# gildas-lormeau/zlib-streams-ts

Measured on NVIDIA B200. Metric: deflate_input_GBps, higher is better.
Workload: dtype u8

## Files before the change

### zlib-streams-ts_b200/csrc/zs_lz77.cu

```cuda
#include <cstdio>
#include <cstdlib>

#include "zs_common.cuh"

namespace {

#ifndef ZS_SEARCH_WARPS
#define ZS_SEARCH_WARPS 30
#endif
#ifndef ZS_HASH_BITS
#define ZS_HASH_BITS 14
#endif
#ifndef ZS_LZ_PREV_POS
#define ZS_LZ_PREV_DELTA 1
#endif
constexpr int kSearchWarps = ZS_SEARCH_WARPS;
constexpr int kWarpParse = kSearchWarps;
constexpr int kWarpInsert = kSearchWarps + 1;
constexpr int kThreads = 32 * (kSearchWarps + 2);
constexpr int kStep = 32 * kSearchWarps;
constexpr unsigned kMaxDist = 32768u - 2u * kStep;
constexpr unsigned kNoPrev = 0xffffu;
constexpr unsigned kSymLimit = 16383u;
constexpr unsigned kTooFar = 4096u;
constexpr unsigned kHashBits = ZS_HASH_BITS;
constexpr unsigned kRing = 65536;
constexpr unsigned kRingGuard = 288;
constexpr unsigned pow2_at_least(unsigned v) { unsigned r = 1; while (r < v) r <<= 1; return r; }
constexpr unsigned kResRing = pow2_at_least(4 * kStep + 64);
constexpr unsigned kMjRing = pow2_at_least(3 * kStep + 64);
constexpr unsigned kPbRing = pow2_at_least(2 * kSearchWarps + 4);
constexpr unsigned kMaxSegChunks = 256;

struct LevelCfg { int lazy_fn, good, lazy, nice, chain; };
__constant__ LevelCfg c_levels[10] = {
    {0, 0, 0, 0, 0},      {0, 4, 4, 8, 4},      {0, 4, 5, 16, 8},      {0, 4, 6, 32, 32},
    {1, 4, 4, 16, 16},    {1, 8, 16, 32, 32},   {1, 8, 16, 128, 128},  {1, 8, 32, 128, 256},
    {1, 32, 128, 258, 1024}, {1, 32, 258, 258, 4096}};

constexpr uint32_t PREP_HAS_PRED = 1u << 21, PREP_LAST = 1u << 22, PREP_VALID = 1u << 23;

struct Smem {
    uint8_t ring[kRing + kRingGuard];
    uint16_t head[1 << kHashBits];
    uint16_t prev[32768];
    uint32_t prep[3 * kStep];
    uint16_t oldh[2 * kStep];
    uint2 pb[kPbRing];
    uint32_t res[kResRing];
    uint2 mj[kMjRing];
    uint32_t bnd[kMaxSegChunks + 1];
    uint32_t seg;
    uint32_t claim[2];
    alignas(8) uint64_t stage_bar;
};
static_assert(sizeof(Smem) <= 227 * 1024, "shared memory budget");

struct LzArgs {
    const uint8_t* buf;
    uint64_t org;
    uint64_t valid_lo;
    uint64_t data_end;
    const uint64_t* in_off;
    uint32_t n_chunks, seg_chunks, n_seg, max_bpc;
    uint32_t n_big, seg_small;
    int level;
    int strategy;
    int cross;
    uint32_t* sym;
    uint32_t* chunk_nblk;
    uint32_t* blk_desc;
    uint32_t* seg_counter;
    int debug;
    unsigned stop_after, stop_active;
};

#ifdef ZS_LZ_PROF
__device__ unsigned long long g_prof[16];
#define PROF_T(i) if (lane == 0) atomicAdd(&g_prof[i], (unsigned long long)(clock64() - t_begin))
#else
#define PROF_T(i)
#endif

__device__ __forceinline__ unsigned res_slot(uint32_t q) { return q & (kResRing - 1u); }
__device__ __forceinline__ unsigned mj_slot(uint32_t q) { return q & (kMjRing - 1u); }

__device__ __forceinline__ uint32_t win32(const Smem& S, uint64_t pos) {
    const unsigned idx = (unsigned)pos & (kRing - 1u);
    const unsigned al = idx & ~3u;
    const uint32_t lo = *reinterpret_cast<const uint32_t*>(S.ring + al);
    const uint32_t hi = *reinterpret_cast<const uint32_t*>(S.ring + al + 4);
    return __funnelshift_r(lo, hi, (idx & 3u) * 8u);
}

__device__ __forceinline__ void stage_window(Smem& S, const LzArgs& a, uint64_t from, uint64_t to, unsigned tid, unsigned nthr) {
    const uint64_t safe16 = (a.data_end + 15) & ~15ull;
    for (uint64_t pos = from + 16ull * tid; pos < to; pos += 16ull * nthr) {
        uint4 v = make_uint4(0, 0, 0, 0);
        if (pos < safe16) v = __ldg(reinterpret_cast<const uint4*>(a.buf + pos));
        const unsigned idx = (unsigned)pos & (kRing - 1u);
        *reinterpret_cast<uint4*>(S.ring + idx) = v;
        if (idx < kRingGuard) *reinterpret_cast<uint4*>(S.ring + kRing + idx) = v;
    }
}

#ifndef ZS_LZ_NO_BULK
#define ZS_LZ_BULK 1
#endif
__device__ __forceinline__ unsigned smem_addr(const void* p) { return (unsigned)__cvta_generic_to_shared(p); }
__device__ __forceinline__ void mbar_init(uint64_t* bar, unsigned count) {
    asm volatile("mbarrier.init.shared::cta.b64 [%0], %1;" ::"r"(smem_addr(bar)), "r"(count) : "memory");
    asm volatile("fence.mbarrier_init.release.cluster;" ::: "memory");
}
__device__ __forceinline__ void mbar_expect_tx(uint64_t* bar, unsigned bytes) {
    asm volatile("mbarrier.arrive.expect_tx.shared::cta.b64 _, [%0], %1;" ::"r"(smem_addr(bar)), "r"(bytes) : "memory");
}
__device__ __forceinline__ void mbar_wait(uint64_t* bar, unsigned parity) {
    asm volatile(
        "{\n"
        ".reg .pred p;\n"
        "ZS_MBAR_WAIT:\n"
        "mbarrier.try_wait.parity.shared::cta.b64 p, [%0], %1;\n"
        "@p bra ZS_MBAR_DONE;\n"
        "bra ZS_MBAR_WAIT;\n"
        "ZS_MBAR_DONE:\n"
        "}\n" ::"r"(smem_addr(bar)), "r"(parity) : "memory");
}
__device__ __forceinline__ void bulk_g2s(void* dst, const void* src, unsigned bytes, uint64_t* bar) {
    asm volatile("cp.async.bulk.shared::cluster.global.mbarrier::complete_tx::bytes [%0], [%1], %2, [%3];" ::"r"(smem_addr(dst)),
                 "l"(src), "r"(bytes), "r"(smem_addr(bar))
                 : "memory");
}
__device__ __forceinline__ unsigned bulk_stage(Smem& S, const uint8_t* buf, uint64_t from, uint64_t to) {
    unsigned total = 0;
    while (from < to) {
        const unsigned idx = (unsigned)from & (kRing - 1u);
        unsigned nb = (unsigned)(to - from);
        if (idx + nb > kRing) nb = kRing - idx;
#ifdef ZS_DEBUG_HOOKS
        if (idx + nb > kRing || (nb & 15u) || (idx & 15u) || ((uintptr_t)(buf + from) & 15u)) { printf("[lz77 bulk] bad copy idx %u nb %u\n", idx, nb); __trap(); }
#endif
        bulk_g2s(S.ring + idx, buf + from, nb, &S.stage_bar);
        total += nb;
        if (idx < kRingGuard) {
            const unsigned g = idx + nb < kRingGuard ? nb : kRingGuard - idx;
#ifdef ZS_DEBUG_HOOKS
            if (idx + g > kRingGuard || (g & 15u)) { printf("[lz77 bulk] bad guard copy idx %u g %u\n", idx, g); __trap(); }
#endif
            bulk_g2s(S.ring + kRing + idx, buf + from, g, &S.stage_bar);
            total += g;
        }
        from += nb;
    }
    return total;
}

__device__ __forceinline__ unsigned hash3(uint32_t w) { return ((w & 0xffffffu) * 0x9E3779B1u) >> (32 - kHashBits); }

struct RangeCtx {
    uint32_t cb;
    uint32_t n;
    uint32_t pre;
    uint32_t tail;
    uint32_t q_data;
    uint32_t nc;
    int cross;
    unsigned min_len;
};

__device__ __forceinline__ uint32_t prep_batch(const Smem& S, const RangeCtx& c, uint32_t q0, uint32_t limit) {
    const unsigned lane = zs_lane();
    const uint32_t q = q0 + lane;
    const bool valid = q < limit && q + 2 < c.tail;
    unsigned h = 0;
    if (valid) h = hash3(win32(S, c.cb + q));
#ifndef ZS_PREP_MATCH_ANY
    unsigned peers = __ballot_sync(ZS_FULL_MASK, valid);
#pragma unroll
    for (int bit = 0; bit < (int)kHashBits; ++bit) {
        const bool one = (h >> bit) & 1u;
        const unsigned bal = __ballot_sync(ZS_FULL_MASK, one);
        peers &= one ? bal : ~bal;
    }
#else
    const unsigned peers = __match_any_sync(ZS_FULL_MASK, valid ? h : 0x10000u + lane);
#endif
    if (!valid) return 0u;
    const unsigned lower = peers & zs_lanemask_lt();
    uint32_t w = h | PREP_VALID;
    if (lower) w |= PREP_HAS_PRED | ((31u - __clz(lower)) << 16);
    if ((peers >> lane) == 1u) w |= PREP_LAST;
    return w;
}

__device__ __forceinline__ void head_exchange(Smem& S, uint32_t p16, uint32_t w, uint16_t* oldh) {
    const unsigned h = w & 0x7fffu;
    unsigned old = 0;
    if ((w & PREP_VALID) && !(w & PREP_HAS_PRED)) old = S.head[h];
    if (w & PREP_LAST) S.head[h] = (uint16_t)(p16 + zs_lane());
    oldh[zs_lane()] = (uint16_t)old;
    __syncwarp();
}
__device__ __forceinline__ void link_batch(Smem& S, const RangeCtx& c, uint32_t q0, uint32_t w, unsigned old) {
    if (w & PREP_VALID) {
        const uint32_t q = q0 + zs_lane();
        const unsigned p16 = (c.cb + q) & 0xffffu;
#ifdef ZS_LZ_PREV_DELTA
        unsigned hop = kNoPrev;
        if (w & PREP_HAS_PRED) {
            hop = zs_lane() - ((w >> 16) & 31u);
        } else {
            const unsigned delta = (p16 - old) & 0xffffu;
            if (delta != 0 && delta <= kMaxDist && delta <= q + c.pre) hop = delta;
        }
        S.prev[p16 & 32767u] = (uint16_t)hop;
#else
        unsigned pred = p16;
        if (w & PREP_HAS_PRED) {
            pred = (c.cb + q0 + ((w >> 16) & 31u)) & 0xffffu;
        } else {
            const unsigned delta = (p16 - old) & 0xffffu;
            if (delta != 0 && delta <= kMaxDist && delta <= q + c.pre) pred = (p16 - delta) & 0xffffu;
        }
        S.prev[p16 & 32767u] = (uint16_t)pred;
#endif
    }
}

#ifdef ZS_LZ_PREV_DELTA
__device__ __forceinline__ bool chain_hop(const Smem& S, unsigned& ci, unsigned& dist, unsigned max_back, unsigned& delta) {
    delta = S.prev[ci & 32767u];
    dist += delta;
    if (dist > max_back) return false;
    ci = (ci - delta) & (kRing - 1u);
    return true;
}
#else
__device__ __forceinline__ bool chain_hop(const Smem& S, unsigned& ci, unsigned& dist, unsigned max_back, unsigned& delta) {
    delta = (ci - S.prev[ci & 32767u]) & 0xffffu;
    if (delta == 0) return false;
    dist += delta;
    if (dist > max_back) return false;
    ci = (ci - delta) & (kRing - 1u);
    return true;
}
#endif

__device__ __forceinline__ uint32_t ring32(const Smem& S, unsigned idx) {
    idx &= kRing - 1u;
    const unsigned al = idx & ~3u;
    const uint32_t lo = *reinterpret_cast<const uint32_t*>(S.ring + al);
    const uint32_t hi = *reinterpret_cast<const uint32_t*>(S.ring + al + 4);
    return __funnelshift_r(lo, hi, (idx & 3u) * 8u);
}
__device__ __forceinline__ unsigned first_diff_byte(uint32_t x) { return (unsigned)(__ffs((int)x) - 1) >> 3; }

__device__ __forceinline__ uint2 ring64(const Smem& S, unsigned idx) {
    idx &= kRing - 1u;
    const unsigned al = idx & ~3u, sh = (idx & 3u) * 8u;
    const uint32_t w0 = *reinterpret_cast<const uint32_t*>(S.ring + al);
    const uint32_t w1 = *reinterpret_cast<const uint32_t*>(S.ring + al + 4);
    const uint32_t w2 = *reinterpret_cast<const uint32_t*>(S.ring + al + 8);
    return make_uint2(__funnelshift_r(w0, w1, sh), __funnelshift_r(w1, w2, sh));
}
__device__ __forceinline__ unsigned extend_match(const Smem& S, unsigned ci, unsigned pi, unsigned len, unsigned max_len) {
    unsigned aa = ((ci + len) & (kRing - 1u)) & ~3u, ab = ((pi + len) & (kRing - 1u)) & ~3u;
    const unsigned sa = ((ci + len) & 3u) * 8u, sb = ((pi + len) & 3u) * 8u;
    uint32_t a0 = *reinterpret_cast<const uint32_t*>(S.ring + aa);
    uint32_t b0 = *reinterpret_cast<const uint32_t*>(S.ring + ab);
// ... 140 lines not shown
    if (best_len < c.min_len) return lit;
    if (best_len == 3 && best_dist > kTooFar) return lit;
    return lit | (best_len << 15) | best_dist;
}

constexpr unsigned MJ_MATCH = 1u << 9;
__device__ __forceinline__ unsigned mj_exit(unsigned y) { return y & 0x1ffu; }
__device__ __forceinline__ unsigned mj_count(unsigned y) { return (y >> 10) & 0x3fu; }
__device__ __forceinline__ unsigned mj_pair_exit(unsigned y) { return ((y >> 16) & 0x1ffu) + 32u; }
__device__ __forceinline__ unsigned mj_pair_count(unsigned y) { return y >> 25; }

template <int kMode>
__device__ __forceinline__ void resolve_one(const Smem& S, const LevelCfg& cfg, uint32_t n, uint32_t q0, unsigned& M,
                                            unsigned& J, bool& is_match) {
    const unsigned lane = zs_lane();
    const uint32_t q = q0 + lane;
    const uint32_t r = q < n ? S.res[res_slot(q)] : 0u;
    const unsigned L = (r >> 15) & 0x1ffu;
    unsigned Ln = __shfl_down_sync(ZS_FULL_MASK, L, 1);
    if (lane == 31) Ln = (q + 1 < n) ? ((S.res[res_slot(q + 1)] >> 15) & 0x1ffu) : 0u;
    const bool deferred = kMode == 1 && L >= 3 && L < (unsigned)cfg.lazy && Ln > L;
    is_match = L >= 3 && !deferred;
    J = q < n ? lane + (is_match ? L : 1u) : 32u;
    M = q < n ? 1u << lane : 0u;
#pragma unroll
    for (int round = 0; round < 5; ++round) {
        const unsigned src = J < 32 ? J : lane;
        const unsigned Mj = __shfl_sync(ZS_FULL_MASK, M, src);
        const unsigned Jj = __shfl_sync(ZS_FULL_MASK, J, src);
        if (J < 32) { M |= Mj; J = Jj; }
    }
}

template <int kMode>
__device__ __forceinline__ void resolve_pair(Smem& S, const LevelCfg& cfg, uint32_t n, uint32_t q0) {
    const unsigned lane = zs_lane();
    unsigned Ma, Ja, Mb, Jb;
    bool ma, mb;
    resolve_one<kMode>(S, cfg, n, q0, Ma, Ja, ma);
    resolve_one<kMode>(S, cfg, n, q0 + 32, Mb, Jb, mb);
    const unsigned ca = __popc(Ma), cb = __popc(Mb);
    const unsigned xa = Ja - 32u;
    const unsigned src = xa < 32u ? xa : lane;
    const unsigned jb = __shfl_sync(ZS_FULL_MASK, Jb, src), cbx = __shfl_sync(ZS_FULL_MASK, cb, src);
    const unsigned pair_exit = xa < 32u ? 32u + jb : Ja;
    const unsigned pair_cnt = xa < 32u ? ca + cbx : ca;
    const unsigned pe = pair_exit >= 32u ? pair_exit - 32u : 0u;
    if (q0 + lane < n)
        S.mj[mj_slot(q0 + lane)] = make_uint2(Ma, Ja | (ma ? MJ_MATCH : 0u) | (ca << 10) | (pe << 16) | (pair_cnt << 25));
    if (q0 + 32 + lane < n)
        S.mj[mj_slot(q0 + 32 + lane)] = make_uint2(Mb, Jb | (mb ? MJ_MATCH : 0u) | (cb << 10));
}

struct ParseState {
    uint32_t ppos;
    uint32_t skip;
    uint32_t nsym;
    uint32_t blk;
    uint32_t blk_sym0;
    uint32_t blk_pos0;
    uint32_t jc;
    uint32_t cstart;
    uint32_t nb;
};

__device__ __forceinline__ void close_block(const LzArgs& a, const RangeCtx& rc, ParseState& ps, uint32_t c0, uint32_t pos_end) {
    if (ps.blk < a.max_bpc && zs_lane() == 0) {
        uint32_t* d = a.blk_desc + ((uint64_t)(c0 + ps.jc) * a.max_bpc + ps.blk) * 4;
        d[0] = ps.blk_sym0 - (ps.cstart - rc.q_data);
        d[1] = ps.nsym - ps.blk_sym0;
        d[2] = ps.blk_pos0 - ps.cstart;
        d[3] = pos_end - ps.blk_pos0;
    }
    ps.blk++;
    ps.blk_sym0 = ps.nsym;
    ps.blk_pos0 = pos_end;
}

__device__ __forceinline__ void close_chunk(const Smem& S, const LzArgs& a, const RangeCtx& rc, ParseState& ps, uint32_t c0) {
    close_block(a, rc, ps, c0, ps.nb);
    if (zs_lane() == 0) a.chunk_nblk[c0 + ps.jc] = ps.blk < a.max_bpc ? ps.blk : a.max_bpc;
    ps.jc++;
    ps.cstart = ps.nb;
    ps.nb = ps.jc < rc.nc ? S.bnd[ps.jc + 1] : 0xffffffffu;
    ps.blk = 0;
}

__device__ __forceinline__ unsigned below(unsigned b) { return b >= 32u ? 0xffffffffu : (1u << b) - 1u; }

constexpr int kParseGroup = 16;
template <bool kBoundary>
__device__ __forceinline__ void parse_group(Smem& S, const LzArgs& a, const RangeCtx& rc, ParseState& ps, uint32_t c0,
                                            uint32_t qb, int np) {
    const unsigned lane = zs_lane();
    const uint32_t n = rc.n;
    unsigned ya[kParseGroup], yb[kParseGroup];
#pragma unroll
    for (int u = 0; u < kParseGroup; ++u) {
        const uint32_t q = qb + 64u * u + lane;
        ya[u] = (u < np && q < n) ? S.mj[mj_slot(q)].y : (32u | (32u << 16));
        yb[u] = (u < np && q + 32 < n) ? S.mj[mj_slot(q + 32)].y : 32u;
    }
#pragma unroll
    for (int u = 0; u < kParseGroup; ++u) {
        if (u < np) {
            const uint32_t q0 = qb + 64u * u;
            unsigned entry = 64u;
            const uint32_t first_sym = ps.nsym;
            if (ps.skip >= 64) {
                ps.skip -= 64;
            } else {
                unsigned s = ps.skip;
                entry = s;
                while (kBoundary && ps.nb < q0 + 64u) {
                    const unsigned b = ps.nb - q0;
                    unsigned c;
                    if (b <= s) {
                        c = 0;
                    } else if (s < 32u) {
                        const uint2 m = S.mj[mj_slot(q0 + s)];
                        c = __popc(m.x & below(b));
                        if (b > 32u) {
                            const unsigned xa = mj_exit(m.y) - 32u;
                            if (xa < b - 32u) c += __popc(S.mj[mj_slot(q0 + 32u + xa)].x & below(b - 32u));
                        }
                    } else {
                        c = __popc(S.mj[mj_slot(q0 + s)].x & below(b - 32u));
                    }
                    if (ps.nsym - ps.blk_sym0 + c > kSymLimit) close_block(a, rc, ps, c0, q0 + s);
                    ps.nsym += c;
                    close_chunk(S, a, rc, ps, c0);
                    s = b;
                }
                const unsigned wa = __shfl_sync(ZS_FULL_MASK, ya[u], s & 31u);
                const unsigned wb = __shfl_sync(ZS_FULL_MASK, yb[u], s & 31u);
                unsigned cnt, exit_rel;
                if (s < 32) { cnt = mj_pair_count(wa); exit_rel = mj_pair_exit(wa); }
                else { cnt = mj_count(wb); exit_rel = 32u + mj_exit(wb); }
                if (ps.nsym - ps.blk_sym0 + cnt > kSymLimit) close_block(a, rc, ps, c0, q0 + s);
                ps.nsym += cnt;
                ps.skip = exit_rel >= 64u ? exit_rel - 64u : 0u;
                while (kBoundary && ps.nb <= q0 + exit_rel) close_chunk(S, a, rc, ps, c0);
            }
            if (lane == 0) S.pb[(q0 >> 6) & (kPbRing - 1u)] = make_uint2(entry, first_sym);
        }
    }
}

__device__ __forceinline__ void emit_batch(const Smem& S, const LzArgs& a, uint64_t sym_base, uint32_t n, uint32_t q0) {
    const unsigned lane = zs_lane();
    const uint2 e = S.pb[(q0 >> 6) & (kPbRing - 1u)];
    if (e.x >= 64u) return;
    unsigned entry, first = e.y;
    if (!(q0 & 32u)) {
        if (e.x >= 32u) return;
        entry = e.x;
    } else if (e.x >= 32u) {
        entry = e.x - 32u;
    } else {
        const unsigned ya = S.mj[mj_slot(q0 - 32u + e.x)].y;
        const unsigned xa = mj_exit(ya) - 32u;
        if (xa >= 32u) return;
        entry = xa;
        first += mj_count(ya);
    }
    if (q0 + entry >= n) return;
    const unsigned visited = S.mj[mj_slot(q0 + entry)].x;
    if (((visited >> lane) & 1u) && q0 + lane < n) {
        const uint32_t q = q0 + lane;
        const uint32_t r = S.res[res_slot(q)];
        const bool is_match = (S.mj[mj_slot(q)].y & MJ_MATCH) != 0;
        a.sym[sym_base + first + __popc(visited & zs_lanemask_lt())] =
            is_match ? (((r & 0x7fffu) << 16) | ((r >> 15) & 0x1ffu)) : (r >> 24);
    }
}

__device__ __forceinline__ uint32_t resolved_frontier(uint32_t searched, uint32_t n) {
    if (searched >= n) return n;
    return searched >= 64 ? (searched - 1) & ~63u : 0;
}

template <int kMode>
__global__ void __launch_bounds__(kThreads, 1) lz77_kernel(LzArgs a) {
    extern __shared__ __align__(16) unsigned char smem_raw[];
    Smem& S = *reinterpret_cast<Smem*>(smem_raw);
    const unsigned wid = threadIdx.x >> 5, lane = zs_lane();
    LevelCfg cfg = c_levels[a.level];
    const StopCfg stop = {a.stop_after, a.stop_active};
    (void)stop;
#ifdef ZS_LZ_PROF
    if (a.debug >> 8) cfg.chain = a.debug >> 8;
#endif

#ifdef ZS_LZ_BULK
    if (threadIdx.x == 0) mbar_init(&S.stage_bar, 1);
#endif
    for (;;) {
        if (threadIdx.x == 0) S.seg = atomicAdd(a.seg_counter, 1u);
        __syncthreads();
        const uint32_t seg = S.seg;
        if (seg >= a.n_seg) break;
        const bool big = seg < a.n_big;
        const uint32_t c0 = big ? seg * a.seg_chunks : a.n_big * a.seg_chunks + (seg - a.n_big) * a.seg_small;
        const uint32_t sc = big ? a.seg_chunks : a.seg_small;
        const uint32_t c1 = (c0 + sc < a.n_chunks) ? c0 + sc : a.n_chunks;

        const uint32_t nc = c1 - c0;

        if (threadIdx.x == 0) S.claim[0] = 0;
        {
            uint4* z = reinterpret_cast<uint4*>(S.head);
            const unsigned nz = (sizeof(S.head) + sizeof(S.prev)) / sizeof(uint4);
#ifdef ZS_LZ_PREV_DELTA
            const unsigned nh = sizeof(S.head) / sizeof(uint4);
            for (unsigned i = threadIdx.x; i < nz; i += kThreads) {
                const unsigned v = i < nh ? 0u : 0xffffffffu;
                z[i] = make_uint4(v, v, v, v);
            }
#else
            for (unsigned i = threadIdx.x; i < nz; i += kThreads) z[i] = make_uint4(0, 0, 0, 0);
#endif
        }
        const uint64_t off0 = a.in_off[c0];
        const uint64_t seg_start = a.org + off0;
        const uint64_t seg_end = a.org + a.in_off[c1];
        uint64_t prime0 = seg_start;
        if (a.cross) {
            prime0 = seg_start > a.valid_lo + 32768 ? seg_start - 32768 : a.valid_lo;
            prime0 = (prime0 + 31) & ~31ull;
            if (prime0 > seg_start) prime0 = seg_start;
        }
        RangeCtx rc;
        rc.cb = (uint32_t)prime0;
        rc.n = (uint32_t)(seg_end - prime0);
        rc.q_data = (uint32_t)(seg_start - prime0);
        rc.nc = nc;
        rc.cross = a.cross;
        rc.min_len = (kMode == 1 && a.strategy == ZS_STRATEGY_FILTERED) ? 6u : 3u;
        {
            const uint64_t pre = a.cross ? prime0 - a.valid_lo : 0;
            rc.pre = pre < kMaxDist ? (uint32_t)pre : kMaxDist;
            const uint64_t tail = a.data_end - prime0;
            rc.tail = tail < 0xffffffffull ? (uint32_t)tail : 0xffffffffu;
        }
        for (unsigned j = threadIdx.x; j <= nc; j += kThreads) S.bnd[j] = (uint32_t)(a.in_off[c0 + j] - off0) + rc.q_data;
        const uint64_t base16 = prime0 & ~15ull;
        const uint32_t p0lo = (uint32_t)prime0 & 15u;
        const uint32_t safe_rel = [&] {
            const uint64_t d = ((a.data_end + 15) & ~15ull) - base16;
            return d < 0xfffffff0ull ? (uint32_t)d : 0xfffffff0u;
        }();
        stage_window(S, a, base16, base16 + ((p0lo + 2u * kStep + kRingGuard + 15u) & ~15u), threadIdx.x, kThreads);
        __syncthreads();

        const uint32_t n = rc.n;
        const uint32_t nsteps = (n + kStep - 1) / kStep;
        const uint32_t n_iter = nsteps + 6;
        const uint32_t nwait = (nsteps + 1u) & ~1u;
        (void)nwait;
        const uint32_t qd64 = rc.q_data & ~63u;
        ParseState ps;
        ps.ppos = qd64; ps.skip = rc.q_data - qd64; ps.nsym = 0; ps.blk = 0; ps.blk_sym0 = 0; ps.blk_pos0 = rc.q_data;
        ps.jc = 0; ps.cstart = rc.q_data; ps.nb = S.bnd[1];
        if (wid == kWarpParse)
            while (ps.nb <= rc.q_data) close_chunk(S, a, rc, ps, c0);
        unsigned js = 0;
        uint32_t cs_w = rc.q_data, ce_w = S.bnd[1];
        uint32_t q_prep = 0;
        unsigned s_prep = 0;
        uint32_t searched = 0;
        uint32_t r0 = qd64, r1 = qd64, r2 = qd64, r3 = qd64;

        for (uint32_t k = 0; k < n_iter; ++k) {
#ifdef ZS_LZ_PROF
            const long long t_begin = clock64();
#endif
            r3 = r2; r2 = r1; r1 = r0;
            r0 = resolved_frontier(searched, n);
            if (r0 < qd64) r0 = qd64;
            const unsigned s_ins = s_prep == 0 ? 2u : s_prep - 1u;
            const unsigned s_link = s_ins == 0 ? 2u : s_ins - 1u;
            if (wid == kWarpInsert) {
                const uint32_t stage_from = (p0lo + q_prep + 2u * kStep + kRingGuard + 15u) & ~15u;
                const uint32_t stage_to = k < nsteps ? (p0lo + q_prep + 3u * kStep + kRingGuard + 15u) & ~15u : stage_from;
#ifdef ZS_LZ_BULK
                const uint32_t bulk_to = stage_to < safe_rel ? stage_to : safe_rel;
                if (k < nwait && lane == 0) {
                    unsigned total = 0;
                    if (stage_from < bulk_to) {
                        asm volatile("fence.proxy.async.shared::cta;" ::: "memory");
                        const unsigned i0 = ((uint32_t)base16 + stage_from) & (kRing - 1u), nb = bulk_to - stage_from;
                        total = nb;
                        if (i0 < kRingGuard) total += (i0 + nb < kRingGuard ? nb : kRingGuard - i0);
                        if (i0 + nb > kRing) total += (i0 + nb - kRing < kRingGuard ? i0 + nb - kRing : kRingGuard);
                    }
                    mbar_expect_tx(&S.stage_bar, total);
                    if (total) bulk_stage(S, a.buf, base16 + stage_from, base16 + bulk_to);
                }
#else
                constexpr int kStageVec = (kStep + 16 + 511) / 512;
                uint4 sv[kStageVec];
#pragma unroll
                for (int v = 0; v < kStageVec; ++v) {
                    const uint32_t pos = stage_from + 16u * (lane + 32 * v);
                    sv[v] = make_uint4(0, 0, 0, 0);
                    if (pos < stage_to && pos < safe_rel) sv[v] = __ldg(reinterpret_cast<const uint4*>(a.buf + base16 + pos));
                }
#endif
                if (k >= 1 && k - 1 < nsteps) {
                    const uint32_t p16 = rc.cb + q_prep - kStep;
                    const uint32_t* pw = S.prep + s_ins * kStep;
                    uint16_t* oh = S.oldh + ((k - 1) & 1u) * kStep;
#pragma unroll 8
                    for (int u = 0; u < kSearchWarps; ++u) head_exchange(S, p16 + 32u * u, pw[32 * u + lane], oh + 32 * u);
                }
#ifdef ZS_LZ_BULK
                if (stage_to > safe_rel) {
                    for (uint32_t pos = (stage_from > safe_rel ? stage_from : safe_rel) + 16u * lane; pos < stage_to; pos += 512u) {
                        const unsigned idx = ((uint32_t)base16 + pos) & (kRing - 1u);
                        *reinterpret_cast<uint4*>(S.ring + idx) = make_uint4(0, 0, 0, 0);
                        if (idx < kRingGuard) *reinterpret_cast<uint4*>(S.ring + kRing + idx) = make_uint4(0, 0, 0, 0);
                    }
                }
#ifdef ZS_LZ_BULK_DEBUG
                if (k < nwait) {
                    unsigned tries = 0, ok = 0;
                    while (!ok && tries < 200000u) {
                        asm volatile("{\n.reg .pred p;\nmbarrier.try_wait.parity.shared::cta.b64 p, [%1], %2;\nselp.u32 %0, 1, 0, p;\n}\n"
                                     : "=r"(ok) : "r"(smem_addr(&S.stage_bar)), "r"(k & 1u) : "memory");
                        ++tries;
                    }
                    if (!ok && lane == 0)
                        printf("[lz77 bulk] wait timed out: cta %u seg %u k %u of %u from %u to %u bulk_to %u safe %u p0lo %u base16 %llu\n",
                               blockIdx.x, seg, k, nsteps, stage_from, stage_to, bulk_to, safe_rel, p0lo, (unsigned long long)base16);
                }
#else
                if (k < nwait) mbar_wait(&S.stage_bar, k & 1u);
#endif
#else
#pragma unroll
                for (int v = 0; v < kStageVec; ++v) {
                    const uint32_t pos = stage_from + 16u * (lane + 32 * v);
                    if (pos < stage_to) {
                        const unsigned idx = ((uint32_t)base16 + pos) & (kRing - 1u);
                        *reinterpret_cast<uint4*>(S.ring + idx) = sv[v];
                        if (idx < kRingGuard) *reinterpret_cast<uint4*>(S.ring + kRing + idx) = sv[v];
                    }
                }
                if (stage_to > stage_from + 512u * kStageVec)
                    stage_window(S, a, base16 + stage_from + 512u * kStageVec, base16 + stage_to, lane, 32);
#endif
            } else if (wid == kWarpParse) {
                while (ps.ppos < r1) {
                    int np = (int)((r1 - ps.ppos + 63) / 64);
                    if (np > kParseGroup) np = kParseGroup;
                    if (ps.nb > ps.ppos + 64u * (unsigned)np + 258u) parse_group<false>(S, a, rc, ps, c0, ps.ppos, np);
                    else parse_group<true>(S, a, rc, ps, c0, ps.ppos, np);
                    ps.ppos += 64u * np;
                }
            } else {
                const unsigned i = wid * 32 + lane;
                if (k < nsteps) {
                    const uint32_t se = q_prep + kStep < n ? q_prep + kStep : n;
                    S.prep[s_prep * kStep + i] = prep_batch(S, rc, q_prep + 32u * wid, se);
                }
                if (k >= 2 && k - 2 < nsteps)
                    link_batch(S, rc, q_prep - 2u * kStep + 32u * wid, S.prep[s_link * kStep + i], S.oldh[(k & 1u) * kStep + i]);
                if (k >= 3 && k - 3 < nsteps) {
                    const uint32_t qw = q_prep - 3u * kStep + 32u * wid;
                    const uint32_t q = qw + lane;
                    if (qw + 32u > qd64 && qw < n) {
                        while (qw >= ce_w) { ++js; cs_w = ce_w; ce_w = S.bnd[js + 1]; }
                        uint32_t r = 0;
                        if constexpr (kMode == 1) {
                            const bool live = q >= rc.q_data && q < n;
                            uint32_t cs = cs_w, ce = ce_w;
                            if (live && q >= ce) {
                                unsigned jl = js;
                                do { ++jl; cs = ce; ce = S.bnd[jl + 1]; } while (q >= ce);
                            }
                            const uint32_t rr = search_lazy_endwin(S, cfg, stop, rc, q, cs, ce, live);
                            r = live ? rr : 0u;
                        } else
                        if (q >= rc.q_data && q < n) {
                            uint32_t cs = cs_w, ce = ce_w;
                            if (q >= ce) {
                                unsigned jl = js;
                                do { ++jl; cs = ce; ce = S.bnd[jl + 1]; } while (q >= ce);
                            }
                            r = search_position<kMode == 1 ? 0 : kMode>(S, cfg, rc, q, cs, ce);
                        }
                        if (q < n) S.res[res_slot(q)] = r;
                    }
                }
                constexpr unsigned kHalf = kSearchWarps / 2;
#ifndef ZS_LZ_NO_CLAIM
                if constexpr (kMode == 1) {
                    const unsigned nr = r0 > r1 ? (r0 - r1 + 63u) >> 6 : 0u, ne = r2 > r3 ? (r2 - r3 + 63u) >> 6 : 0u;
                    if (threadIdx.x == 0) S.claim[(k + 1u) & 1u] = 0;
                    for (;;) {
                        unsigned item = 0;
                        if (lane == 0) item = atomicAdd(&S.claim[k & 1u], 1u);
                        item = __shfl_sync(ZS_FULL_MASK, item, 0);
                        if (item >= nr + ne) break;
                        if (item < nr) {
                            resolve_pair<kMode>(S, cfg, n, r1 + 64u * item);
                        } else {
                            const uint32_t q0 = r3 + 64u * (item - nr);
                            emit_batch(S, a, off0, n, q0);
                            if (q0 + 32 < r2) emit_batch(S, a, off0, n, q0 + 32);
                        }
                    }
                } else
#endif
                if (wid < kHalf) {
                    for (uint32_t q0 = r1 + 64u * wid; q0 < r0; q0 += 64u * kHalf) resolve_pair<kMode>(S, cfg, n, q0);
                } else {
                    for (uint32_t q0 = r3 + 64u * (wid - kHalf); q0 < r2; q0 += 64u * (kSearchWarps - kHalf)) {
                        emit_batch(S, a, off0, n, q0);
                        if (q0 + 32 < r2) emit_batch(S, a, off0, n, q0 + 32);
                    }
                }
            }
#ifdef ZS_LZ_PROF
            {
                const long long t_work = clock64() - t_begin;
                __syncwarp();
                if (lane == 0) {
                    const int role = wid == kWarpInsert ? 0 : wid == kWarpParse ? 1 : 2;
                    atomicAdd(&g_prof[role], (unsigned long long)t_work);
                    if (wid == 0) atomicAdd(&g_prof[4], 1ull);
                }
            }
#endif
            if (k >= 3) searched = searched + kStep < n ? searched + kStep : n;
            q_prep += kStep;
            s_prep = s_prep == 2 ? 0u : s_prep + 1u;
            __syncthreads();
#ifdef ZS_LZ_PROF
            if (threadIdx.x == 0) atomicAdd(&g_prof[3], (unsigned long long)(clock64() - t_begin));
#endif
        }
        if (wid == kWarpParse)
            while (ps.jc < nc) close_chunk(S, a, rc, ps, c0);
        __syncthreads();
    }
}

__global__ void plain_blocks_kernel(LzArgs a, uint32_t per_block, int with_symbols) {
    const uint32_t c = blockIdx.x * blockDim.x + threadIdx.x;
    if (c >= a.n_chunks) return;
    const uint32_t n = (uint32_t)(a.in_off[c + 1] - a.in_off[c]);
    uint32_t nb = (n + per_block - 1) / per_block;
    if (nb == 0) nb = 1;
    if (nb > a.max_bpc) nb = a.max_bpc;
    for (uint32_t j = 0; j < nb; j++) {
        uint32_t* d = a.blk_desc + ((uint64_t)c * a.max_bpc + j) * 4;
        const uint32_t b0 = j * per_block, len = n - b0 < per_block ? n - b0 : per_block;
        d[0] = with_symbols ? b0 : 0u;
        d[1] = with_symbols ? len : 0u;
        d[2] = b0;
        d[3] = len;
    }
    a.chunk_nblk[c] = nb;
}
__global__ void literal_symbols_kernel(const uint8_t* in, uint32_t* sym, uint64_t n) {
    for (uint64_t i = (uint64_t)blockIdx.x * blockDim.x + threadIdx.x; i < n; i += (uint64_t)gridDim.x * blockDim.x) sym[i] = in[i];
}

}

int zs_launch_lz77(zs_ctx* ctx, const zs_deflate_plan& p) {
    static bool attr_set[64] = {false};
    const int dev_slot = ctx->device >= 0 && ctx->device < 64 ? ctx->device : 0;
    if (!attr_set[dev_slot] || ctx->device >= 64) {
        ZS_CUDA_TRY(ctx, cudaFuncSetAttribute(lz77_kernel<0>, cudaFuncAttributeMaxDynamicSharedMemorySize, (int)sizeof(Smem)));
        ZS_CUDA_TRY(ctx, cudaFuncSetAttribute(lz77_kernel<1>, cudaFuncAttributeMaxDynamicSharedMemorySize, (int)sizeof(Smem)));
        ZS_CUDA_TRY(ctx, cudaFuncSetAttribute(lz77_kernel<2>, cudaFuncAttributeMaxDynamicSharedMemorySize, (int)sizeof(Smem)));
        attr_set[dev_slot] = true;
    }
    LzArgs a;
    const uintptr_t first = reinterpret_cast<uintptr_t>(p.d_in) - p.history;
    const uintptr_t adj = first & 15u;
    a.buf = reinterpret_cast<const uint8_t*>(first - adj);
    a.valid_lo = adj;
    a.org = adj + p.history;
    a.data_end = a.org + p.in_len;
    a.in_off = p.d_in_off;
    a.n_chunks = p.n_chunks;
    a.max_bpc = p.max_bpc;
    a.level = p.level;
    a.strategy = p.strategy;
    a.cross = (p.mode == ZS_MODE_STITCHED || (p.flags & ZS_FLAG_PRIME)) ? 1 : 0;
    uint32_t seg_chunks = 1;
    if (a.cross) {
        seg_chunks = p.n_chunks / (4u * (uint32_t)ctx->sm_count);
        if (seg_chunks < 1) seg_chunks = 1;
        if (seg_chunks > 16) seg_chunks = 16;
    } else {
        uint64_t waves = p.in_len / ((uint64_t)ctx->sm_count * (512u << 10));
        if (waves < 1) waves = 1;
        const uint64_t want = waves * (uint64_t)ctx->sm_count;
        uint64_t sc = (p.n_chunks + want - 1) / want;
        if (sc < 1) sc = 1;
        if (sc > kMaxSegChunks) sc = kMaxSegChunks;
        seg_chunks = (uint32_t)sc;
    }
    if (a.cross && p.seg_hint) seg_chunks = p.seg_hint < kMaxSegChunks ? p.seg_hint : kMaxSegChunks;
    a.seg_chunks = seg_chunks;
    a.seg_small = seg_chunks >= 4 ? seg_chunks / 4 : 1;
    a.n_big = (uint32_t)(((uint64_t)p.n_chunks * 3 / 4) / seg_chunks);
    {
        const uint32_t rest = p.n_chunks - a.n_big * seg_chunks;
        a.n_seg = a.n_big + (rest + a.seg_small - 1) / a.seg_small;
    }
    a.sym = p.d_sym;
    a.chunk_nblk = p.d_chunk_nblk;
    a.blk_desc = p.d_blk_desc;
    a.seg_counter = p.d_seg_counter;
    a.debug = 0;
    a.stop_after = 8;
    a.stop_active = 8;
    if (const char* e = getenv("ZS_LZ_STOP_AFTER")) a.stop_after = (unsigned)atoi(e);
    if (const char* e = getenv("ZS_LZ_STOP_ACTIVE")) a.stop_active = (unsigned)atoi(e);
#ifdef ZS_LZ_PROF
    if (getenv("ZS_LZ_DEBUG")) a.debug = atoi(getenv("ZS_LZ_DEBUG"));
#endif
// ... 41 lines not shown
```

Baseline: 27.75.

## Split LZ77 kernel into per-role loops and fuse hash-peer ballot via PTX

Restructures the per-segment step loop so the insert warp, parse warp and search warps each run their own specialised loop function, synchronised by a raw bar.sync barrier instead of one shared loop that branches on warp role every step. This is meant to cut per-role register pressure and branch overhead and let each role keep only its own state. It also replaces the per-bit ballot/select in prep_batch with inline PTX that fuses the predicate, vote and lop3 mask, and moves the chunk count into shared memory. The risk is that the role loops must keep exactly matching iteration counts for the barrier to stay correct.

New measurement: 29.78, median of 6. 1.07x the previous value.

```diff
diff --git a/zlib-streams-ts_b200/csrc/zs_lz77.cu b/zlib-streams-ts_b200/csrc/zs_lz77.cu
--- a/zlib-streams-ts_b200/csrc/zs_lz77.cu
+++ b/zlib-streams-ts_b200/csrc/zs_lz77.cu
@@ -51,6 +51,7 @@
     uint2 mj[kMjRing];
     uint32_t bnd[kMaxSegChunks + 1];
     uint32_t seg;
+    uint32_t nc;
     uint32_t claim[2];
     alignas(8) uint64_t stage_bar;
 };
@@ -77,7 +78,7 @@
 
 #ifdef ZS_LZ_PROF
 __device__ unsigned long long g_prof[16];
-#define PROF_T(i) if (lane == 0) atomicAdd(&g_prof[i], (unsigned long long)(clock64() - t_begin))
+#define PROF_T(i) { const long long t_work = clock64() - t_begin; __syncwarp(); if (lane == 0) atomicAdd(&g_prof[i], (unsigned long long)t_work); }
 #else
 #define PROF_T(i)
 #endif
@@ -163,10 +164,24 @@
     uint32_t pre;
     uint32_t tail;
     uint32_t q_data;
-    uint32_t nc;
     int cross;
     unsigned min_len;
 };
+
+__device__ __forceinline__ unsigned peers_bit(unsigned peers, unsigned h, unsigned bit_mask) {
+    unsigned r;
+    asm("{\n"
+        ".reg .pred p;\n"
+        ".reg .b32 t, bal, m;\n"
+        "and.b32 t, %1, %3;\n"
+        "setp.ne.u32 p, t, 0;\n"
+        "vote.sync.ballot.b32 bal, p, 0xffffffff;\n"
+        "selp.b32 m, -1, 0, p;\n"
+        "lop3.b32 %0, %2, bal, m, 0x90;\n"
+        "}\n"
+        : "=r"(r) : "r"(h), "r"(peers), "r"(bit_mask));
+    return r;
+}
 
 __device__ __forceinline__ uint32_t prep_batch(const Smem& S, const RangeCtx& c, uint32_t q0, uint32_t limit) {
     const unsigned lane = zs_lane();
@@ -174,17 +189,9 @@
     const bool valid = q < limit && q + 2 < c.tail;
     unsigned h = 0;
     if (valid) h = hash3(win32(S, c.cb + q));
-#ifndef ZS_PREP_MATCH_ANY
     unsigned peers = __ballot_sync(ZS_FULL_MASK, valid);
 #pragma unroll
-    for (int bit = 0; bit < (int)kHashBits; ++bit) {
-        const bool one = (h >> bit) & 1u;
-        const unsigned bal = __ballot_sync(ZS_FULL_MASK, one);
-        peers &= one ? bal : ~bal;
-    }
-#else
-    const unsigned peers = __match_any_sync(ZS_FULL_MASK, valid ? h : 0x10000u + lane);
-#endif
+    for (int bit = 0; bit < (int)kHashBits; ++bit) peers = peers_bit(peers, h, 1u << bit);
     if (!valid) return 0u;
     const unsigned lower = peers & zs_lanemask_lt();
     uint32_t w = h | PREP_VALID;
@@ -491,7 +498,7 @@
     if (zs_lane() == 0) a.chunk_nblk[c0 + ps.jc] = ps.blk < a.max_bpc ? ps.blk : a.max_bpc;
     ps.jc++;
     ps.cstart = ps.nb;
-    ps.nb = ps.jc < rc.nc ? S.bnd[ps.jc + 1] : 0xffffffffu;
+    ps.nb = ps.jc < S.nc ? S.bnd[ps.jc + 1] : 0xffffffffu;
     ps.blk = 0;
 }
 
@@ -589,14 +596,228 @@
     return searched >= 64 ? (searched - 1) & ~63u : 0;
 }
 
+__device__ __forceinline__ void step_barrier() { asm volatile("bar.sync 0, %0;" ::"n"(kThreads) : "memory"); }
+
+__device__ __forceinline__ void insert_loop(Smem& S, const LzArgs& a, const RangeCtx& rc, uint32_t nsteps, uint64_t base16,
+                                            uint32_t p0lo, uint32_t safe_rel) {
+    const unsigned lane = zs_lane();
+    const uint32_t n_iter = nsteps + 6;
+    const uint32_t nwait = (nsteps + 1u) & ~1u;
+    (void)nwait;
+    uint32_t stage_end = p0lo + 2u * kStep + kRingGuard + 15u;
+    uint32_t p16 = rc.cb - kStep;
+    unsigned s_ins = 2;
+    for (uint32_t k = 0; k < n_iter; ++k) {
+#ifdef ZS_LZ_PROF
+        const long long t_begin = clock64();
+#endif
+        const uint32_t stage_from = stage_end & ~15u;
+        const uint32_t stage_to = k < nsteps ? (stage_end + kStep) & ~15u : stage_from;
+#ifdef ZS_LZ_BULK
+        const uint32_t bulk_to = stage_to < safe_rel ? stage_to : safe_rel;
+        if (k < nwait && lane == 0) {
+            unsigned total = 0;
+            if (stage_from < bulk_to) {
+                asm volatile("fence.proxy.async.shared::cta;" ::: "memory");
+                const unsigned i0 = ((uint32_t)base16 + stage_from) & (kRing - 1u), nb = bulk_to - stage_from;
+                total = nb;
+                if (i0 < kRingGuard) total += (i0 + nb < kRingGuard ? nb : kRingGuard - i0);
+                if (i0 + nb > kRing) total += (i0 + nb - kRing < kRingGuard ? i0 + nb - kRing : kRingGuard);
+            }
+            mbar_expect_tx(&S.stage_bar, total);
+            if (total) bulk_stage(S, a.buf, base16 + stage_from, base16 + bulk_to);
+        }
+#else
+        constexpr int kStageVec = (kStep + 16 + 511) / 512;
+        uint4 sv[kStageVec];
+#pragma unroll
+        for (int v = 0; v < kStageVec; ++v) {
+            const uint32_t pos = stage_from + 16u * (lane + 32 * v);
+            sv[v] = make_uint4(0, 0, 0, 0);
+            if (pos < stage_to && pos < safe_rel) sv[v] = __ldg(reinterpret_cast<const uint4*>(a.buf + base16 + pos));
+        }
+#endif
+        if (k - 1u < nsteps) {
+            const uint32_t* pw = S.prep + s_ins * kStep;
+            uint16_t* oh = S.oldh + ((k - 1u) & 1u) * kStep;
+#pragma unroll 8
+            for (int u = 0; u < kSearchWarps; ++u) head_exchange(S, p16 + 32u * u, pw[32 * u + lane], oh + 32 * u);
+        }
+#ifdef ZS_LZ_BULK
+        if (stage_to > safe_rel) {
+            for (uint32_t pos = (stage_from > safe_rel ? stage_from : safe_rel) + 16u * lane; pos < stage_to; pos += 512u) {
+                const unsigned idx = ((uint32_t)base16 + pos) & (kRing - 1u);
+                *reinterpret_cast<uint4*>(S.ring + idx) = make_uint4(0, 0, 0, 0);
+                if (idx < kRingGuard) *reinterpret_cast<uint4*>(S.ring + kRing + idx) = make_uint4(0, 0, 0, 0);
+            }
+        }
+#ifdef ZS_LZ_BULK_DEBUG
+        if (k < nwait) {
+            unsigned tries = 0, ok = 0;
+            while (!ok && tries < 200000u) {
+                asm volatile("{\n.reg .pred p;\nmbarrier.try_wait.parity.shared::cta.b64 p, [%1], %2;\nselp.u32 %0, 1, 0, p;\n}\n"
+                             : "=r"(ok) : "r"(smem_addr(&S.stage_bar)), "r"(k & 1u) : "memory");
+                ++tries;
+            }
+            if (!ok && lane == 0)
+                printf("[lz77 bulk] wait timed out: cta %u seg %u k %u of %u from %u to %u bulk_to %u safe %u p0lo %u base16 %llu\n",
+                       blockIdx.x, S.seg, k, nsteps, stage_from, stage_to, bulk_to, safe_rel, p0lo, (unsigned long long)base16);
+        }
+#else
+        if (k < nwait) mbar_wait(&S.stage_bar, k & 1u);
+#endif
+#else
+#pragma unroll
+        for (int v = 0; v < kStageVec; ++v) {
+            const uint32_t pos = stage_from + 16u * (lane + 32 * v);
+            if (pos < stage_to) {
+                const unsigned idx = ((uint32_t)base16 + pos) & (kRing - 1u);
+                *reinterpret_cast<uint4*>(S.ring + idx) = sv[v];
+                if (idx < kRingGuard) *reinterpret_cast<uint4*>(S.ring + kRing + idx) = sv[v];
+            }
+        }
+        if (stage_to > stage_from + 512u * kStageVec)
+            stage_window(S, a, base16 + stage_from + 512u * kStageVec, base16 + stage_to, lane, 32);
+#endif
+        PROF_T(0);
+        step_barrier();
+        stage_end += kStep;
+        p16 += kStep;
+        s_ins = s_ins == 2 ? 0u : s_ins + 1u;
+    }
+}
+
+__device__ __forceinline__ void parse_loop(Smem& S, const LzArgs& a, const RangeCtx& rc, uint32_t c0, uint32_t nsteps) {
+    const unsigned lane = zs_lane();
+    (void)lane;
+    const uint32_t n = rc.n;
+    const uint32_t qd64 = rc.q_data & ~63u;
+    ParseState ps;
+    ps.ppos = qd64; ps.skip = rc.q_data - qd64; ps.nsym = 0; ps.blk = 0; ps.blk_sym0 = 0; ps.blk_pos0 = rc.q_data;
+    ps.jc = 0; ps.cstart = rc.q_data; ps.nb = S.bnd[1];
+    while (ps.nb <= rc.q_data) close_chunk(S, a, rc, ps, c0);
+    const uint32_t end = (nsteps + 6) * kStep;
+    for (uint32_t kq = 0; kq < end; kq += kStep) {
+#ifdef ZS_LZ_PROF
+        const long long t_begin = clock64();
+#endif
+        const uint32_t searched = kq - 4u * kStep;
+        const uint32_t r1 = kq <= 4u * kStep ? 0u : searched >= n ? n : searched - 64u;
+        while (ps.ppos < r1) {
+            int np = (int)((r1 - ps.ppos + 63) / 64);
+            if (np > kParseGroup) np = kParseGroup;
+            if (ps.nb > ps.ppos + 64u * (unsigned)np + 258u) parse_group<false>(S, a, rc, ps, c0, ps.ppos, np);
+            else parse_group<true>(S, a, rc, ps, c0, ps.ppos, np);
+            ps.ppos += 64u * np;
+        }
+        PROF_T(1);
+        step_barrier();
+    }
+    while (ps.jc < S.nc) close_chunk(S, a, rc, ps, c0);
+}
+
+template <int kMode>
+__device__ __forceinline__ void wide_loop(Smem& S, const LzArgs& a, const LevelCfg& cfg, const RangeCtx& rc, uint64_t off0,
+                                          uint32_t nsteps) {
+    const unsigned wid = threadIdx.x >> 5, lane = zs_lane();
+    const unsigned i = threadIdx.x;
+    const StopCfg stop = {a.stop_after, a.stop_active};
+    (void)stop;
+    const uint32_t n = rc.n, n_iter = nsteps + 6;
+    const uint32_t qd64 = rc.q_data & ~63u;
+    unsigned js = 0;
+    uint32_t cs_w = rc.q_data, ce_w = S.bnd[1];
+    uint32_t qb = 32u * wid;
+    uint32_t qe = kStep;
+    unsigned o_prep = 0;
+    uint32_t searched = 0;
+    uint32_t r0 = qd64, r1 = qd64, r2 = qd64, r3 = qd64;
+    for (uint32_t k = 0; k < n_iter; ++k) {
+#ifdef ZS_LZ_PROF
+        const long long t_begin = clock64();
+#endif
+        r3 = r2; r2 = r1; r1 = r0;
+        r0 = resolved_frontier(searched, n);
+        if (r0 < qd64) r0 = qd64;
+        const unsigned o_link = o_prep == 2u * kStep ? 0u : o_prep + kStep;
+        if (k < nsteps) S.prep[o_prep + i] = prep_batch(S, rc, qb, qe < n ? qe : n);
+        if (k - 2u < nsteps) link_batch(S, rc, qb - 2u * kStep, S.prep[o_link + i], S.oldh[(k & 1u) * kStep + i]);
+        if (k - 3u < nsteps) {
+            const uint32_t qw = qb - 3u * kStep;
+            const uint32_t q = qw + lane;
+            if (qw + 32u > qd64 && qw < n) {
+                while (qw >= ce_w) { ++js; cs_w = ce_w; ce_w = S.bnd[js + 1]; }
+                uint32_t r = 0;
+                if constexpr (kMode == 1) {
+                    const bool live = q >= rc.q_data && q < n;
+                    uint32_t cs = cs_w, ce = ce_w;
+                    if (live && q >= ce) {
+                        unsigned jl = js;
+                        do { ++jl; cs = ce; ce = S.bnd[jl + 1]; } while (q >= ce);
+                    }
+                    const uint32_t rr = search_lazy_endwin(S, cfg, stop, rc, q, cs, ce, live);
+                    r = live ? rr : 0u;
+                } else
+                if (q >= rc.q_data && q < n) {
+                    uint32_t cs = cs_w, ce = ce_w;
+                    if (q >= ce) {
+                        unsigned jl = js;
+                        do { ++jl; cs = ce; ce = S.bnd[jl + 1]; } while (q >= ce);
+                    }
+                    r = search_position<kMode == 1 ? 0 : kMode>(S, cfg, rc, q, cs, ce);
+                }
+                if (q < n) S.res[res_slot(q)] = r;
+            }
+        }
+        constexpr unsigned kHalf = kSearchWarps / 2;
+#ifndef ZS_LZ_NO_CLAIM
+        if constexpr (kMode == 1) {
+            const unsigned nr = r0 > r1 ? (r0 - r1 + 63u) >> 6 : 0u, ne = r2 > r3 ? (r2 - r3 + 63u) >> 6 : 0u;
+            if (i == 0) S.claim[(k + 1u) & 1u] = 0;
+            for (;;) {
+                unsigned item = 0;
+                if (lane == 0) item = atomicAdd(&S.claim[k & 1u], 1u);
+                item = __shfl_sync(ZS_FULL_MASK, item, 0);
+                if (item >= nr + ne) break;
+                if (item < nr) {
+                    resolve_pair<kMode>(S, cfg, n, r1 + 64u * item);
+                } else {
+                    const uint32_t q0 = r3 + 64u * (item - nr);
+                    emit_batch(S, a, off0, n, q0);
+                    if (q0 + 32 < r2) emit_batch(S, a, off0, n, q0 + 32);
+                }
+            }
+        } else
+#endif
+        if (wid < kHalf) {
+            for (uint32_t q0 = r1 + 64u * wid; q0 < r0; q0 += 64u * kHalf) resolve_pair<kMode>(S, cfg, n, q0);
+        } else {
+            for (uint32_t q0 = r3 + 64u * (wid - kHalf); q0 < r2; q0 += 64u * (kSearchWarps - kHalf)) {
+                emit_batch(S, a, off0, n, q0);
+                if (q0 + 32 < r2) emit_batch(S, a, off0, n, q0 + 32);
+            }
+        }
+        PROF_T(2);
+#ifdef ZS_LZ_PROF
+        if (i == 0) atomicAdd(&g_prof[4], 1ull);
+#endif
+        if (k >= 3) searched = searched + kStep < n ? searched + kStep : n;
+        qb += kStep;
+        qe += kStep;
+        o_prep = o_link;
+        step_barrier();
+#ifdef ZS_LZ_PROF
+        if (i == 0) atomicAdd(&g_prof[3], (unsigned long long)(clock64() - t_begin));
+#endif
+    }
+}
+
 template <int kMode>
 __global__ void __launch_bounds__(kThreads, 1) lz77_kernel(LzArgs a) {
     extern __shared__ __align__(16) unsigned char smem_raw[];
     Smem& S = *reinterpret_cast<Smem*>(smem_raw);
-    const unsigned wid = threadIdx.x >> 5, lane = zs_lane();
+    const unsigned wid = threadIdx.x >> 5;
     LevelCfg cfg = c_levels[a.level];
-    const StopCfg stop = {a.stop_after, a.stop_active};
-    (void)stop;
 #ifdef ZS_LZ_PROF
     if (a.debug >> 8) cfg.chain = a.debug >> 8;
 #endif
@@ -616,7 +837,7 @@
 
         const uint32_t nc = c1 - c0;
 
-        if (threadIdx.x == 0) S.claim[0] = 0;
+        if (threadIdx.x == 0) { S.claim[0] = 0; S.nc = nc; }
         {
             uint4* z = reinterpret_cast<uint4*>(S.head);
             const unsigned nz = (sizeof(S.head) + sizeof(S.prev)) / sizeof(uint4);
@@ -643,7 +864,6 @@
         rc.cb = (uint32_t)prime0;
         rc.n = (uint32_t)(seg_end - prime0);
         rc.q_data = (uint32_t)(seg_start - prime0);
-        rc.nc = nc;
         rc.cross = a.cross;
         rc.min_len = (kMode == 1 && a.strategy == ZS_STRATEGY_FILTERED) ? 6u : 3u;
         {
@@ -655,203 +875,18 @@
         for (unsigned j = threadIdx.x; j <= nc; j += kThreads) S.bnd[j] = (uint32_t)(a.in_off[c0 + j] - off0) + rc.q_data;
         const uint64_t base16 = prime0 & ~15ull;
         const uint32_t p0lo = (uint32_t)prime0 & 15u;
-        const uint32_t safe_rel = [&] {
-            const uint64_t d = ((a.data_end + 15) & ~15ull) - base16;
-            return d < 0xfffffff0ull ? (uint32_t)d : 0xfffffff0u;
-        }();
         stage_window(S, a, base16, base16 + ((p0lo + 2u * kStep + kRingGuard + 15u) & ~15u), threadIdx.x, kThreads);
         __syncthreads();
 
-        const uint32_t n = rc.n;
-        const uint32_t nsteps = (n + kStep - 1) / kStep;
-        const uint32_t n_iter = nsteps + 6;
-        const uint32_t nwait = (nsteps + 1u) & ~1u;
-        (void)nwait;
-        const uint32_t qd64 = rc.q_data & ~63u;
-        ParseState ps;
-        ps.ppos = qd64; ps.skip = rc.q_data - qd64; ps.nsym = 0; ps.blk = 0; ps.blk_sym0 = 0; ps.blk_pos0 = rc.q_data;
-        ps.jc = 0; ps.cstart = rc.q_data; ps.nb = S.bnd[1];
-        if (wid == kWarpParse)
-            while (ps.nb <= rc.q_data) close_chunk(S, a, rc, ps, c0);
-        unsigned js = 0;
-        uint32_t cs_w = rc.q_data, ce_w = S.bnd[1];
-        uint32_t q_prep = 0;
-        unsigned s_prep = 0;
-        uint32_t searched = 0;
-        uint32_t r0 = qd64, r1 = qd64, r2 = qd64, r3 = qd64;
-
-        for (uint32_t k = 0; k < n_iter; ++k) {
-#ifdef ZS_LZ_PROF
-            const long long t_begin = clock64();
-#endif
-            r3 = r2; r2 = r1; r1 = r0;
-            r0 = resolved_frontier(searched, n);
-            if (r0 < qd64) r0 = qd64;
-            const unsigned s_ins = s_prep == 0 ? 2u : s_prep - 1u;
-            const unsigned s_link = s_ins == 0 ? 2u : s_ins - 1u;
-            if (wid == kWarpInsert) {
-                const uint32_t stage_from = (p0lo + q_prep + 2u * kStep + kRingGuard + 15u) & ~15u;
-                const uint32_t stage_to = k < nsteps ? (p0lo + q_prep + 3u * kStep + kRingGuard + 15u) & ~15u : stage_from;
-#ifdef ZS_LZ_BULK
-                const uint32_t bulk_to = stage_to < safe_rel ? stage_to : safe_rel;
-                if (k < nwait && lane == 0) {
-                    unsigned total = 0;
-                    if (stage_from < bulk_to) {
-                        asm volatile("fence.proxy.async.shared::cta;" ::: "memory");
-                        const unsigned i0 = ((uint32_t)base16 + stage_from) & (kRing - 1u), nb = bulk_to - stage_from;
-                        total = nb;
-                        if (i0 < kRingGuard) total += (i0 + nb < kRingGuard ? nb : kRingGuard - i0);
-                        if (i0 + nb > kRing) total += (i0 + nb - kRing < kRingGuard ? i0 + nb - kRing : kRingGuard);
-                    }
-                    mbar_expect_tx(&S.stage_bar, total);
-                    if (total) bulk_stage(S, a.buf, base16 + stage_from, base16 + bulk_to);
-                }
-#else
-                constexpr int kStageVec = (kStep + 16 + 511) / 512;
-                uint4 sv[kStageVec];
-#pragma unroll
-                for (int v = 0; v < kStageVec; ++v) {
-                    const uint32_t pos = stage_from + 16u * (lane + 32 * v);
-                    sv[v] = make_uint4(0, 0, 0, 0);
-                    if (pos < stage_to && pos < safe_rel) sv[v] = __ldg(reinterpret_cast<const uint4*>(a.buf + base16 + pos));
-                }
-#endif
-                if (k >= 1 && k - 1 < nsteps) {
-                    const uint32_t p16 = rc.cb + q_prep - kStep;
-                    const uint32_t* pw = S.prep + s_ins * kStep;
-                    uint16_t* oh = S.oldh + ((k - 1) & 1u) * kStep;
-#pragma unroll 8
-                    for (int u = 0; u < kSearchWarps; ++u) head_exchange(S, p16 + 32u * u, pw[32 * u + lane], oh + 32 * u);
-                }
-#ifdef ZS_LZ_BULK
-                if (stage_to > safe_rel) {
-                    for (uint32_t pos = (stage_from > safe_rel ? stage_from : safe_rel) + 16u * lane; pos < stage_to; pos += 512u) {
-                        const unsigned idx = ((uint32_t)base16 + pos) & (kRing - 1u);
-                        *reinterpret_cast<uint4*>(S.ring + idx) = make_uint4(0, 0, 0, 0);
-                        if (idx < kRingGuard) *reinterpret_cast<uint4*>(S.ring + kRing + idx) = make_uint4(0, 0, 0, 0);
-                    }
-                }
-#ifdef ZS_LZ_BULK_DEBUG
-                if (k < nwait) {
-                    unsigned tries = 0, ok = 0;
-                    while (!ok && tries < 200000u) {
-                        asm volatile("{\n.reg .pred p;\nmbarrier.try_wait.parity.shared::cta.b64 p, [%1], %2;\nselp.u32 %0, 1, 0, p;\n}\n"
-                                     : "=r"(ok) : "r"(smem_addr(&S.stage_bar)), "r"(k & 1u) : "memory");
-                        ++tries;
-                    }
-                    if (!ok && lane == 0)
-                        printf("[lz77 bulk] wait timed out: cta %u seg %u k %u of %u from %u to %u bulk_to %u safe %u p0lo %u base16 %llu\n",
-                               blockIdx.x, seg, k, nsteps, stage_from, stage_to, bulk_to, safe_rel, p0lo, (unsigned long long)base16);
-                }
-#else
-                if (k < nwait) mbar_wait(&S.stage_bar, k & 1u);
-#endif
-#else
-#pragma unroll
-                for (int v = 0; v < kStageVec; ++v) {
-                    const uint32_t pos = stage_from + 16u * (lane + 32 * v);
-                    if (pos < stage_to) {
-                        const unsigned idx = ((uint32_t)base16 + pos) & (kRing - 1u);
-                        *reinterpret_cast<uint4*>(S.ring + idx) = sv[v];
-                        if (idx < kRingGuard) *reinterpret_cast<uint4*>(S.ring + kRing + idx) = sv[v];
-                    }
-                }
-                if (stage_to > stage_from + 512u * kStageVec)
-                    stage_window(S, a, base16 + stage_from + 512u * kStageVec, base16 + stage_to, lane, 32);
-#endif
-            } else if (wid == kWarpParse) {
-                while (ps.ppos < r1) {
-                    int np = (int)((r1 - ps.ppos + 63) / 64);
-                    if (np > kParseGroup) np = kParseGroup;
-                    if (ps.nb > ps.ppos + 64u * (unsigned)np + 258u) parse_group<false>(S, a, rc, ps, c0, ps.ppos, np);
-                    else parse_group<true>(S, a, rc, ps, c0, ps.ppos, np);
-                    ps.ppos += 64u * np;
-                }
-            } else {
-                const unsigned i = wid * 32 + lane;
-                if (k < nsteps) {
-                    const uint32_t se = q_prep + kStep < n ? q_prep + kStep : n;
-                    S.prep[s_prep * kStep + i] = prep_batch(S, rc, q_prep + 32u * wid, se);
-                }
-                if (k >= 2 && k - 2 < nsteps)
-                    link_batch(S, rc, q_prep - 2u * kStep + 32u * wid, S.prep[s_link * kStep + i], S.oldh[(k & 1u) * kStep + i]);
-                if (k >= 3 && k - 3 < nsteps) {
-                    const uint32_t qw = q_prep - 3u * kStep + 32u * wid;
-                    const uint32_t q = qw + lane;
-                    if (qw + 32u > qd64 && qw < n) {
-                        while (qw >= ce_w) { ++js; cs_w = ce_w; ce_w = S.bnd[js + 1]; }
-                        uint32_t r = 0;
-                        if constexpr (kMode == 1) {
-                            const bool live = q >= rc.q_data && q < n;
-                            uint32_t cs = cs_w, ce = ce_w;
-                            if (live && q >= ce) {
-                                unsigned jl = js;
-                                do { ++jl; cs = ce; ce = S.bnd[jl + 1]; } while (q >= ce);
-                            }
-                            const uint32_t rr = search_lazy_endwin(S, cfg, stop, rc, q, cs, ce, live);
-                            r = live ? rr : 0u;
-                        } else
-                        if (q >= rc.q_data && q < n) {
-                            uint32_t cs = cs_w, ce = ce_w;
-                            if (q >= ce) {
-                                unsigned jl = js;
-                                do { ++jl; cs = ce; ce = S.bnd[jl + 1]; } while (q >= ce);
-                            }
-                            r = search_position<kMode == 1 ? 0 : kMode>(S, cfg, rc, q, cs, ce);
-                        }
-                        if (q < n) S.res[res_slot(q)] = r;
-                    }
-                }
-                constexpr unsigned kHalf = kSearchWarps / 2;
-#ifndef ZS_LZ_NO_CLAIM
-                if constexpr (kMode == 1) {
-                    const unsigned nr = r0 > r1 ? (r0 - r1 + 63u) >> 6 : 0u, ne = r2 > r3 ? (r2 - r3 + 63u) >> 6 : 0u;
-                    if (threadIdx.x == 0) S.claim[(k + 1u) & 1u] = 0;
-                    for (;;) {
-                        unsigned item = 0;
-                        if (lane == 0) item = atomicAdd(&S.claim[k & 1u], 1u);
-                        item = __shfl_sync(ZS_FULL_MASK, item, 0);
-                        if (item >= nr + ne) break;
-                        if (item < nr) {
-                            resolve_pair<kMode>(S, cfg, n, r1 + 64u * item);
-                        } else {
-                            const uint32_t q0 = r3 + 64u * (item - nr);
-                            emit_batch(S, a, off0, n, q0);
-                            if (q0 + 32 < r2) emit_batch(S, a, off0, n, q0 + 32);
-                        }
-                    }
-                } else
-#endif
-                if (wid < kHalf) {
-                    for (uint32_t q0 = r1 + 64u * wid; q0 < r0; q0 += 64u * kHalf) resolve_pair<kMode>(S, cfg, n, q0);
-                } else {
-                    for (uint32_t q0 = r3 + 64u * (wid - kHalf); q0 < r2; q0 += 64u * (kSearchWarps - kHalf)) {
-                        emit_batch(S, a, off0, n, q0);
-                        if (q0 + 32 < r2) emit_batch(S, a, off0, n, q0 + 32);
-                    }
-                }
-            }
-#ifdef ZS_LZ_PROF
-            {
-                const long long t_work = clock64() - t_begin;
-                __syncwarp();
-                if (lane == 0) {
-                    const int role = wid == kWarpInsert ? 0 : wid == kWarpParse ? 1 : 2;
-                    atomicAdd(&g_prof[role], (unsigned long long)t_work);
-                    if (wid == 0) atomicAdd(&g_prof[4], 1ull);
-                }
-            }
-#endif
-            if (k >= 3) searched = searched + kStep < n ? searched + kStep : n;
-            q_prep += kStep;
-            s_prep = s_prep == 2 ? 0u : s_prep + 1u;
-            __syncthreads();
-#ifdef ZS_LZ_PROF
-            if (threadIdx.x == 0) atomicAdd(&g_prof[3], (unsigned long long)(clock64() - t_begin));
-#endif
-        }
-        if (wid == kWarpParse)
-            while (ps.jc < nc) close_chunk(S, a, rc, ps, c0);
+        const uint32_t nsteps = (rc.n + kStep - 1) / kStep;
+        if (wid == kWarpInsert) {
+            const uint64_t d = ((a.data_end + 15) & ~15ull) - base16;
+            insert_loop(S, a, rc, nsteps, base16, p0lo, d < 0xfffffff0ull ? (uint32_t)d : 0xfffffff0u);
+        } else if (wid == kWarpParse) {
+            parse_loop(S, a, rc, c0, nsteps);
+        } else {
+            wide_loop<kMode>(S, a, cfg, rc, off0, nsteps);
+        }
         __syncthreads();
     }
 }
```
